# miloknowles/adaptive-stereo-icra-2021

Measured on AMD Instinct MI355X. Metric: stereo pairs/sec (fwd+adapt-step), KITTI 1242x375 D=192, higher is better.
Workload: dtype f32

## Files before the change

adaptive-stereo-icra-2021_amd/adaptive_stereo/_native.py:

```python
import ctypes
import os

import torch

_HERE = os.path.dirname(os.path.abspath(__file__))
LIB_PATH = os.path.join(_HERE, "libadaptive_stereo_hip.so")
BUILD_HINT = "build it with: make -C %s" % os.path.join(os.path.dirname(_HERE), "csrc")

c_int, c_float, c_i64, c_vp = ctypes.c_int, ctypes.c_float, ctypes.c_int64, ctypes.c_void_p


class Pcl(ctypes.Structure):
  _fields_ = [(n, ctypes.c_int32) for n in ("B", "D", "H", "W", "pd", "ph", "pw")]

  def numel(self):
    return self.B * (self.D + 2 * self.pd) * (self.H + 2 * self.ph) * (self.W + 2 * self.pw) * 32

  def voxels(self):
    return self.B * self.D * self.H * self.W

  def key(self):
    return (self.B, self.D, self.H, self.W, self.pd, self.ph, self.pw)


# ... 4 lines not shown
    return self.kd * self.kh * self.kw


class BnMerge(ctypes.Structure):
  _fields_ = [(n, c_vp) for n in ("stat_mean", "stat_m2", "stat_cnt", "gamma", "beta", "running_mean", "running_var",
                                 "save_mean", "save_invstd", "scale", "shift")] + \
             [("nparts", ctypes.c_int32), ("momentum", c_float), ("eps", c_float)]


class TrunkBn(ctypes.Structure):
  _fields_ = [(n, c_vp) for n in ("stat_mean", "stat_m2", "stat_cnt", "gamma", "beta", "state")] + \
             [("nparts", ctypes.c_int32), ("eps", c_float)]


_P = ctypes.POINTER
_SIGNATURES = {
  "as_last_error": (ctypes.c_char_p, []),
  "as_version": (c_int, []),
  "as_pcl_numel": (c_i64, [_P(Pcl)]),
  "as_cost_volume_fwd": (c_int, [c_vp, c_vp, c_vp, _P(Pcl), c_vp]),
  "as_cost_volume_bwd": (c_int, [c_vp, c_vp, c_vp, _P(Pcl), c_vp]),
  "as_conv32_pack_weights": (c_int, [c_vp, c_vp, _P(ConvShape), c_int, c_vp]),
  "as_conv32_pack_weights_batch": (c_int, [c_vp, c_int, c_int, c_vp]),
  "as_conv32_num_blocks": (c_int, [_P(Pcl)]),
  "as_conv32_stat_parts": (c_int, [_P(Pcl), _P(Pcl), _P(ConvShape)]),
  "as_conv32_fwd": (c_int, [c_vp, _P(Pcl), c_vp, c_vp, c_vp, _P(Pcl), _P(ConvShape), c_int, c_vp, c_vp, c_float,
                            c_vp, c_vp, c_vp, c_vp, c_vp]),
  "as_conv32_dgrad_s2_workspace": (c_i64, []),
  "as_conv32_dgrad_s2": (c_int, [c_vp, _P(Pcl), c_vp, c_vp, _P(Pcl), c_vp, c_vp]),
  "as_conv32_dgrad_s2_pack": (c_int, [c_vp, c_vp, c_vp]),
  "as_conv32_dgrad_s2_packed": (c_int, [c_vp, _P(Pcl), c_vp, c_vp, _P(Pcl), c_vp]),
  "as_conv32_wgrad_workspace": (c_i64, [_P(Pcl), _P(Pcl), _P(ConvShape)]),
  "as_conv32_wgrad": (c_int, [c_vp, _P(Pcl), c_vp, _P(Pcl), _P(ConvShape), c_vp, c_vp, c_int, c_vp, c_vp]),
  "as_bn_finalize": (c_int, [c_vp, c_vp, c_vp, c_int, c_vp, c_vp, c_vp, c_vp, c_float, c_float, c_vp, c_vp, c_vp,
                             c_vp, c_vp]),
  "as_bn_eval_affine": (c_int, [c_vp, c_vp, c_vp, c_vp, c_float, c_vp, c_vp, c_vp, c_vp, c_vp]),
  "as_bn_eval_affine_batch": (c_int, [c_vp, c_int, c_float, c_vp]),
  "as_bn_act_fwd": (c_int, [c_vp, c_vp, c_vp, c_float, c_vp, c_vp, _P(Pcl), c_vp]),
  "as_bn_bwd_workspace": (c_i64, [_P(Pcl)]),
  "as_bn_act_bwd": (c_int, [c_vp, c_vp, c_vp, c_vp, c_vp, c_vp, c_vp, c_float, c_int, c_vp, c_vp, c_vp, c_int, c_vp,
                            _P(Pcl), c_vp]),
  "as_bn_act_bwd_given": (c_int, [c_vp, c_vp, c_vp, c_vp, c_vp, c_vp, c_vp, c_float, c_int, c_vp, c_vp, c_vp, c_int, c_vp,
                                  _P(Pcl), c_int, c_vp]),
  "as_bn_bwd_coef_offset": (c_i64, []),
  "as_bn_bwd_sums": (c_int, [c_vp, c_vp, c_vp, c_vp, c_vp, c_float, c_vp, _P(Pcl), c_int, c_vp, c_vp]),
  "as_bn_bwd_finalize_synced": (c_int, [c_vp, c_vp, c_vp, c_vp, c_vp, c_vp, c_int, c_vp, c_vp]),
  "as_bn_bwd_apply": (c_int, [c_vp, c_vp, c_vp, c_vp, c_vp, c_float, c_vp, c_vp, _P(Pcl), c_vp]),
  "as_conv32_wgrad_bnapply_ok": (c_int, [_P(Pcl), _P(Pcl), _P(ConvShape)]),
  "as_conv32_wgrad_bnapply": (c_int, [c_vp, _P(Pcl), c_vp, c_vp, _P(Pcl), _P(ConvShape), c_vp, c_vp, c_vp, c_vp, c_float,
                                      c_vp, c_vp, c_vp, c_int, c_vp, c_vp]),
  "as_conv32to1_bnsums_ok": (c_int, [_P(Pcl), _P(ConvShape)]),
  "as_conv32to1_bnsums_parts": (c_int, [_P(Pcl)]),
  "as_conv32to1_dgrad_bnsums": (c_int, [c_vp, _P(Pcl), _P(ConvShape), c_vp, c_vp, c_vp, c_vp, c_vp, c_vp, c_float, c_vp, c_vp]),
  "as_wgrad_defer": (c_int, [c_int]),
  "as_wgrad_defer_pending": (c_int, []),
  "as_wgrad_defer_flush": (c_int, [c_vp]),
  "as_conv32_act_ok": (c_int, [_P(Pcl), _P(Pcl), _P(ConvShape)]),
  "as_conv32_act_parts": (c_int, []),
  "as_conv32_act_fwd": (c_int, [c_vp, c_vp, c_vp, c_vp, c_vp, _P(Pcl), c_vp, c_vp, c_float, c_vp, _P(Pcl), _P(ConvShape), c_vp, c_vp,
                                c_vp, c_vp]),
  "as_conv32_wino_ok": (c_int, [_P(Pcl), _P(Pcl), _P(ConvShape)]),
  "as_conv32_wino_parts": (c_int, []),
  "as_conv32_wino_pack_weights": (c_int, [c_vp, c_vp, c_int, c_vp]),
  "as_conv32_wino_fwd": (c_int, [c_vp, c_vp, c_vp, c_vp, c_vp, _P(Pcl), c_vp, c_vp, c_float, c_vp, _P(Pcl), _P(ConvShape), c_vp, c_vp,
                                 c_vp, c_vp]),
  "as_conv32_wino_eval": (c_int, [c_vp, _P(Pcl), _P(ConvShape), c_vp, c_vp, c_vp, c_vp, c_float, c_int, c_vp, c_vp]),
  "as_conv32_wino_bwd_data": (c_int, [c_vp, c_vp, _P(Pcl), _P(ConvShape), c_vp, c_vp, c_vp, c_vp, c_vp, c_float, c_vp, c_vp, c_vp, c_vp,
                                      c_vp, c_vp, c_vp, c_vp]),
  "as_conv32_wino_bwd_filter": (c_int, [c_vp, c_vp, _P(Pcl), _P(ConvShape), c_vp, c_vp, c_int, c_vp, c_vp]),
  "as_conv32_wino_bwd_parts": (c_int, []),
  "as_conv32_wino_bwd_workspace": (c_i64, []),
  "as_conv32_wino_bwd_generation": (c_int, [c_int]),
  "as_conv32_wino_bwd": (c_int, [c_vp, _P(Pcl), c_vp, c_vp, _P(Pcl), _P(ConvShape), c_vp, c_vp, c_vp, c_vp, c_vp, c_float, c_vp,
                                 c_vp, c_vp, c_vp, c_vp, c_vp, c_vp, c_vp, c_int, c_vp, c_vp, c_vp]),
  "as_conv32_wino_bwd_fused_parts": (c_int, []),
  "as_conv32_wino_bwd_fused_workspace": (c_i64, []),
  "as_conv32_wino_bwd_fused": (c_int, [c_vp, _P(Pcl), c_vp, c_vp, _P(Pcl), _P(ConvShape), c_vp, c_vp, c_vp, c_vp, c_vp, c_float, c_vp,
                                       c_vp, c_vp, c_vp, c_vp, c_vp, c_vp, c_int, c_vp, c_vp, c_vp]),
  "as_conv3d_wgrad_lds_assignment": (c_int, [c_int, c_int, c_int, c_vp, c_vp, c_vp]),
  "as_conv32_s2_enable": (c_int, [c_int]),
  "as_conv4_s2_enable": (c_int, [c_int]),
  "as_refine_out_ok": (c_int, [_P(Pcl)]),
  "as_refine_out_fwd": (c_int, [c_vp, c_vp, c_vp, c_vp, c_float, c_vp, _P(Pcl), c_vp, c_vp, c_vp, c_int, c_vp, c_vp]),
  "as_conv32_bwd_fused_ok": (c_int, [_P(Pcl), _P(Pcl), _P(ConvShape)]),
  "as_conv32_bwd_fused_parts": (c_int, []),
  "as_conv32_bwd_fused_workspace": (c_i64, []),
  "as_conv32_bwd_fused": (c_int, [c_vp, _P(Pcl), c_vp, c_vp, _P(Pcl), _P(ConvShape), c_vp, c_vp, c_vp, c_vp, c_vp, c_float, c_vp, c_vp,
                                  c_vp, c_vp, c_vp, c_vp, c_vp, c_int, c_vp, c_vp, c_vp]),
  "as_conv32_bnbwd_parts": (c_int, [_P(Pcl), _P(Pcl), _P(ConvShape)]),
  "as_conv32_fwd_bnbwd": (c_int, [c_vp, _P(Pcl), c_vp, c_vp, _P(Pcl), _P(ConvShape), c_vp, c_vp, c_vp, c_vp, c_vp, c_float,
                                  c_vp, c_vp]),
  "as_agg3d_ok": (c_int, [_P(Pcl)]),
  "as_agg3d_parts": (c_int, [_P(Pcl)]),
  "as_agg3d_fwd": (c_int, [c_vp, _P(Pcl), c_vp, c_vp, c_vp, c_vp, _P(BnMerge), c_vp, c_vp, c_int, c_vp, c_vp, c_float, c_vp, c_vp,
                           c_vp, c_vp]),
  "as_trunk_parts": (c_int, [_P(Pcl), c_int]),
  "as_trunk_fwd": (c_int, [c_vp, c_vp, _P(TrunkBn), c_vp, _P(Pcl), c_int, c_vp, c_vp, c_float, c_vp, c_vp, c_vp, c_vp, c_vp]),
  "as_trunk_finish_fwd": (c_int, [c_vp, _P(Pcl), c_vp, c_vp, c_int, c_int, _P(c_vp), _P(c_vp), c_float, c_vp]),
  "as_trunk_begin_bwd": (c_int, [c_vp, c_vp, c_int, _P(Pcl), c_vp, c_vp]),
  "as_trunk_bwd_workspace": (c_i64, [_P(Pcl), c_int]),
  "as_trunk_bwd": (c_int, [c_vp, c_vp, c_vp, c_vp, c_int, c_vp, c_vp, c_vp, c_vp, c_vp, c_vp, c_vp, c_vp, _P(Pcl), c_int, c_float,
                           c_vp, c_vp, c_int, c_vp, c_vp]),
  "as_trunk_finish_bwd": (c_int, [c_vp, c_int, c_int, _P(c_vp), _P(c_vp), c_int, c_vp]),
  "as_agg_tail_ok": (c_int, [_P(Pcl)]),
  "as_agg_tail_fwd": (c_int, [c_vp, _P(Pcl), c_vp, c_vp, _P(BnMerge), c_vp, c_vp, c_vp, c_float, c_vp, c_vp, c_vp, c_vp, c_vp]),
  "as_conv3d_out_fwd": (c_int, [c_vp, _P(Pcl), c_vp, c_vp, c_vp, c_vp]),
  "as_conv3d_out_bwd_workspace": (c_i64, [_P(Pcl)]),
  "as_conv3d_out_bwd": (c_int, [c_vp, c_vp, _P(Pcl), c_vp, c_vp, c_vp, c_vp, c_int, c_vp, c_vp]),
  "as_conv32to1_fwd": (c_int, [c_vp, _P(Pcl), _P(ConvShape), c_vp, c_vp, c_vp, c_int, c_vp, c_vp]),
  "as_conv32to1_bwd_workspace": (c_i64, [_P(Pcl), _P(ConvShape)]),
  "as_conv32to1_bwd": (c_int, [c_vp, c_vp, _P(Pcl), _P(ConvShape), c_vp, c_vp, c_vp, c_vp, c_int, c_vp, c_vp]),
  "as_pcl4_numel": (c_i64, [_P(Pcl)]),
  "as_pack_in4": (c_int, [c_vp, c_vp, c_int, c_vp, _P(Pcl), c_vp]),
  "as_conv4_pack_weights": (c_int, [c_vp, c_int, c_vp, _P(ConvShape), c_vp]),
  "as_conv4_wgrad_bnapply_ok": (c_int, [_P(Pcl), _P(Pcl), _P(ConvShape)]),
  "as_conv4_wgrad_bnapply_proj": (c_int, [c_vp, _P(Pcl), c_vp, c_vp, _P(Pcl), _P(ConvShape), c_int, c_vp, c_vp, c_vp, c_vp, c_float,
                                          c_vp, c_vp, c_vp, c_vp, c_int, c_vp, c_vp]),
  "as_tap_gather": (c_int, [c_vp, c_vp, c_vp, c_int, c_int, c_int, c_vp]),
  "as_conv4_wgrad_bnapply": (c_int, [c_vp, _P(Pcl), c_vp, c_vp, _P(Pcl), _P(ConvShape), c_int, c_vp, c_vp, c_vp, c_vp, c_float,
                                     c_vp, c_vp, c_vp, c_int, c_vp, c_vp]),
  "as_conv4_stat_parts": (c_int, [_P(Pcl), _P(Pcl), _P(ConvShape)]),
  "as_conv4_fwd": (c_int, [c_vp, _P(Pcl), c_vp, c_vp, c_vp, _P(Pcl), _P(ConvShape), c_int, c_vp, c_vp, c_float,
                           c_vp, c_vp, c_vp, c_vp]),
  "as_conv4_wgrad_workspace": (c_i64, [_P(Pcl), _P(ConvShape)]),
  "as_conv4_wgrad": (c_int, [c_vp, _P(Pcl), c_vp, _P(Pcl), _P(ConvShape), c_int, c_vp, c_vp, c_int, c_vp, c_vp]),
  "as_softargmax_fwd": (c_int, [c_vp, c_int, c_int, c_int, c_int, c_vp, c_vp, c_vp, c_vp]),
  "as_softargmax_bwd": (c_int, [c_vp, c_vp, c_vp, c_int, c_int, c_int, c_int, c_vp, c_vp]),
  "as_agg_tail_bwd_ok": (c_int, [_P(Pcl)]),
  "as_agg_tail_bwd_workspace": (c_i64, [_P(Pcl)]),
  "as_agg_tail_bwd": (c_int, [c_vp, c_vp, c_vp, c_vp, _P(Pcl), c_vp, c_vp, c_vp, c_vp, c_int, c_vp, c_vp]),
  "as_upsample_bilinear_fwd": (c_int, [c_vp, c_int, c_int, c_int, c_vp, c_int, c_int, c_float, c_vp]),
  "as_upsample_bilinear_bwd": (c_int, [c_vp, c_int, c_int, c_int, c_vp, c_int, c_int, c_float, c_vp]),
  "as_warp_fwd": (c_int, [c_vp, c_vp, c_int, c_int, c_int, c_int, c_int, c_vp, c_vp, c_vp]),
  "as_warp_nearest_fwd": (c_int, [c_vp, c_vp, c_int, c_int, c_int, c_int, c_int, c_vp, c_vp, c_vp]),
  "as_warp_bwd": (c_int, [c_vp, c_vp, c_vp, c_int, c_int, c_int, c_int, c_int, c_vp, c_vp]),
  "as_warp_bwd_add": (c_int, [c_vp, c_vp, c_vp, c_vp, c_int, c_int, c_int, c_int, c_int, c_vp, c_vp]),
  "as_monodepth_loss_bwd_masked": (c_int, [c_vp, c_vp, c_vp, c_vp, c_vp, c_vp, c_vp, c_int, c_int, c_int, c_float, c_vp, c_vp, c_vp,
                                           c_vp, c_vp]),
  "as_monodepth_workspace": (c_i64, [c_int, c_int, c_int]),
  "as_monodepth_loss_fwd": (c_int, [c_vp, c_vp, c_vp, c_int, c_int, c_int, c_float, c_vp, c_vp, c_vp, c_vp, c_vp,
                                    c_vp]),
  "as_monodepth_loss_bwd": (c_int, [c_vp, c_vp, c_vp, c_vp, c_vp, c_vp, c_vp, c_int, c_int, c_int, c_float, c_vp,
                                    c_vp, c_vp, c_vp]),
  "as_photometric_chain_workspace": (c_i64, [c_int, c_int, c_int]),
  "as_photometric_chain_fwd": (c_int, [c_vp, c_vp, c_vp, c_int, c_int, c_int, c_float, c_vp, c_vp, c_vp, c_vp, c_vp]),
  "as_photometric_chain_bwd": (c_int, [c_vp, c_vp, c_vp, c_vp, c_vp, c_vp, c_int, c_int, c_int, c_float, c_vp, c_vp, c_vp, c_vp]),
  "as_monodepth_loss_rows_fwd": (c_int, [c_vp, c_vp, c_vp, c_int, c_int, c_int, c_float, c_vp, c_vp, c_vp, c_vp, c_vp, c_vp]),
  "as_masked_sum_workspace": (c_i64, [c_i64]),
  "as_masked_sum": (c_int, [c_vp, c_vp, c_i64, c_vp, c_vp, c_vp]),
  "as_masked_sum_mean": (c_int, [c_vp, c_vp, c_i64, c_vp, c_vp, c_vp]),
  "as_khamis_workspace": (c_i64, [c_i64]),
  "as_khamis_fwd": (c_int, [c_vp, c_vp, c_i64, c_vp, c_vp, c_vp]),
  "as_khamis_bwd": (c_int, [c_vp, c_vp, c_vp, c_vp, c_i64, c_vp, c_vp]),
  "as_eval_metrics_workspace": (c_i64, [c_i64]),
  "as_eval_metrics": (c_int, [c_vp, c_vp, c_i64, c_vp, c_vp, c_vp]),
  "as_relu_bwd": (c_int, [c_vp, c_vp, c_i64, c_vp, c_vp]),
  "as_mirror_taps_ch0": (c_int, [c_vp, c_int, c_vp, c_vp, c_vp]),
  "as_sumsq_workspace": (c_i64, [c_i64]),
  "as_clip_coef": (c_int, [c_vp, c_float, c_vp, c_vp]),
  "as_sumsq_clip": (c_int, [c_vp, c_i64, c_float, c_vp, c_vp, c_vp, c_vp, c_vp]),
  "as_sumsq": (c_int, [c_vp, c_i64, c_vp, c_vp, c_vp]),
  "as_adam_step": (c_int, [c_vp, c_vp, c_vp, c_vp, c_i64, c_vp, c_float, c_float, c_float, c_float, c_int, c_vp,
                           c_vp]),
  "as_decode_rgb8": (c_int, [c_vp, c_int, c_int, c_int, c_int, c_int, c_int, c_int, c_vp, c_vp]),
  "as_decode_plane": (c_int, [c_vp, c_int, c_int, c_int, c_int, c_int, c_int, c_int, c_int, c_int, c_float, c_int, c_vp,
                              c_vp]),
# ... 62 lines not shown
```

adaptive-stereo-icra-2021_amd/adaptive_stereo/hip_ops.py:

```python
import os
import torch

from . import _native as nat
from ._native import Pcl, ConvShape, call, ptr, stream, f32c

LEAKY_SLOPE = 0.2
BN_EPS = 1e-5
BN_MOMENTUM = 0.1

CONV3D_333 = ConvShape(3, 3, 3, 1, 1, 1, 1, 1)

_DIRECT_GRADS = True


def set_direct_grad_accumulation(flag: bool):
  global _DIRECT_GRADS
  _DIRECT_GRADS = bool(flag)


def grad_sinks(params):
  if not (_DIRECT_GRADS and torch.is_grad_enabled()):
    return None
  out = []
  for p in params:
# ... 52 lines not shown

  def put(self, buf, g: Pcl, channels=32):
    if buf is None:
      return
    self.free.setdefault(self._key(buf.device, g, channels), []).append(buf)

  def clear(self):
    self.free.clear()


POOL = PclPool()


class _RmwOrder(object):
  enabled = False
  last = {}
  streams = {}


def rmw_order_reset(enabled):
  if not enabled:
    flush_deferred_reductions()
  _RmwOrder.enabled = bool(enabled)
  _RmwOrder.last = {}
  _RmwOrder.streams = {}
  if enabled and _DEFER_REDUCE and torch.cuda.is_available():
    lib = nat.load()
    if lib.as_wgrad_defer_pending() != 0 or _DeferredReduce.keep:
      raise RuntimeError("adaptive_stereo: a multi-stream region opens while weight-gradient reductions of an earlier one "
                         "are still pending (a region was left without rmw_order_reset(False))")
    _DeferredReduce.on = True
    lib.as_wgrad_defer(1)


class _DeferredReduce(object):
  on = False
  keep = []


_DEFER_REDUCE = True


def set_defer_reduce(enabled):
  global _DEFER_REDUCE
  prev, _DEFER_REDUCE = _DEFER_REDUCE, bool(enabled)
  return prev


def _keep_for_deferred_reduce(ws):
  if _DeferredReduce.on:
    _DeferredReduce.keep.append(ws)


def flush_deferred_reductions():
  join_region_streams()
  if not _DeferredReduce.on:
    return
  lib = nat.load()
  lib.as_wgrad_defer(0)
  _DeferredReduce.on = False
  call("as_wgrad_defer_flush", stream())
  _DeferredReduce.keep = []


_TAIL_BNSUMS = True
_HEAD_PROJ = True
_FWD_ACT = True
_WINOGRAD = os.environ.get("AS_DIAG_DIRECT_FORM") != "1"


def set_tail_bnsums(enabled):
  global _TAIL_BNSUMS
  prev, _TAIL_BNSUMS = _TAIL_BNSUMS, bool(enabled)
  return prev


def set_head_proj(enabled):
  global _HEAD_PROJ
  prev, _HEAD_PROJ = _HEAD_PROJ, bool(enabled)
  return prev


_REFINE_OUT = True


def set_refine_out(enabled):
  global _REFINE_OUT
  prev, _REFINE_OUT = _REFINE_OUT, bool(enabled)
  return prev


def set_head_staged(enabled):
  lib = nat.load()
  prev = lib.as_conv32_s2_enable(2) == 1 and lib.as_conv4_s2_enable(2) == 1
  lib.as_conv32_s2_enable(1 if enabled else 0)
  lib.as_conv4_s2_enable(1 if enabled else 0)
  return prev


def set_fwd_act(enabled):
  global _FWD_ACT
  prev, _FWD_ACT = _FWD_ACT, bool(enabled)
  return prev


_WINOGRAD_BWD = True
_WINOGRAD_BWD_ONE_LAUNCH = True


def set_winograd_bwd_one_launch(flag: bool):
  global _WINOGRAD_BWD_ONE_LAUNCH
  prev, _WINOGRAD_BWD_ONE_LAUNCH = _WINOGRAD_BWD_ONE_LAUNCH, bool(flag)
  return prev


def set_winograd(enabled, backward=None):
  global _WINOGRAD, _WINOGRAD_BWD
  prev, _WINOGRAD = _WINOGRAD, bool(enabled)
  _WINOGRAD_BWD = bool(enabled if backward is None else backward)
  return prev


class _Beside(object):
  enabled = os.environ.get("AS_WGRAD_BESIDE", "0") == "1"
  stream = None
  origin = None
  forks = 0


def set_wgrad_beside(flag: bool):
  prev, _Beside.enabled = _Beside.enabled, bool(flag)
  return prev


def set_fork_origin(handle):
  prev, _Beside.origin = _Beside.origin, handle
  return prev


def fork_beside(fn):
  main = torch.cuda.current_stream()
  if (not _Beside.enabled or _BN_SYNC is not None or
      (torch.cuda.is_current_stream_capturing() and main.cuda_stream != _Beside.origin)):
    fn()
    return None
  if _Beside.stream is None:
    _Beside.stream = torch.cuda.Stream()
  side = _Beside.stream
  side.wait_stream(main)
  with torch.cuda.stream(side):
    fn()
  ev = torch.cuda.Event()
  ev.record(side)
  _Beside.forks += 1
  return ev


def join_beside(ev):
  if ev is not None:
    torch.cuda.current_stream().wait_event(ev)


def _rmw_wait(t):
  if _RmwOrder.enabled and t is not None:
    last = _RmwOrder.last.get(t.data_ptr())
    cur = torch.cuda.current_stream()
    if last is not None and last[0] != cur.cuda_stream:
      cur.wait_event(last[1])


def _rmw_done(t):
# ... 1034 lines not shown
           ptr(stats.mean), ptr(stats.m2), ptr(stats.cnt), stream())
      st0 = bn_train_stats(stats, gamma0, beta0, rm0, rv0)
      fused_act = _FWD_ACT and need_bwd and all(lib.as_conv32_act_ok(g, g, conv_shape_2d(d)) == 1 for d in REFINE_DILATIONS)
      a0 = None if fused_act else bn_act(z0, st0, g)
    else:
      fused_act = False
      st0 = bn_eval_stats(gamma0, beta0, rm0, rv0)
      if need_bwd:
        z0 = POOL.get(g, dev)
        call("as_conv4_fwd", ptr(in4), g4, ptr(wp4), ptr(b0), ptr(z0), g, s33, 0, None, None, LEAKY_SLOPE, None, None,
             None, stream())
        a0 = bn_act(z0, st0, g)
      else:
        z0 = None
        a0 = POOL.get(g, dev)
        call("as_conv4_fwd", ptr(in4), g4, ptr(wp4), ptr(b0), ptr(a0), g, s33, 1, ptr(st0.scale), ptr(st0.shift),
             LEAKY_SLOPE, None, None, None, stream())
    if not need_bwd and z0 is not None:
      POOL.put(z0, g); z0 = None

    xs, zs, sts = [a0], [], []
    tail_fused = None
    if fused_act:
      xs = []
      z_prev, st_prev = z0, st0
      for l, dil in enumerate(REFINE_DILATIONS):
        wl, bl, gamma, beta = params[4 + 4 * l:8 + 4 * l]
        rm, rv = bn_buffers[1 + l]
        a_prev, z, st = block_forward_act(z_prev, xs[-1] if xs else None, st_prev, g, conv_shape_2d(dil), wl, bl, gamma, beta,
                                          rm, rv)
        xs.append(a_prev); zs.append(z); sts.append(st)
        z_prev, st_prev = z, st
      if _REFINE_OUT and lib.as_refine_out_ok(g) == 1:
        tail_fused = (z_prev, xs[-1], st_prev)
      else:
        xs.append(bn_act(z_prev, st_prev, g, residual=xs[-1]))
    else:
      for l, dil in enumerate(REFINE_DILATIONS):
        wl, bl, gamma, beta = params[4 + 4 * l:8 + 4 * l]
        rm, rv = bn_buffers[1 + l]
        z, a, st = block_forward(xs[-1], g, conv_shape_2d(dil), wl, bl, gamma, beta, rm, rv, train, True, need_bwd)
        zs.append(z); sts.append(st); xs.append(a)
        if not need_bwd:
          POOL.put(xs[-2], g)

    w_out, b_out = params[28], params[29]
    out = torch.empty(B, 1, H, W, dtype=torch.float32, device=dev)
    if tail_fused is not None:
      z6, a5, st6 = tail_fused
      a6 = POOL.get(g, dev)
      call("as_refine_out_fwd", ptr(z6), ptr(a5), ptr(st6.scale), ptr(st6.shift), LEAKY_SLOPE, ptr(a6), g, ptr(w_out), ptr(b_out),
           ptr(up), 1, ptr(out), stream())
      xs.append(a6)
    elif _REFINE_OUT and lib.as_refine_out_ok(g) == 1:
      call("as_refine_out_fwd", ptr(xs[-1]), None, None, None, LEAKY_SLOPE, None, g, ptr(w_out), ptr(b_out), ptr(up), 1, ptr(out),
           stream())
    else:
      call("as_conv32to1_fwd", ptr(xs[-1]), g, s33, ptr(w_out), ptr(b_out), ptr(up), 1, ptr(out), stream())

    if need_bwd:
      ctx.g, ctx.g4, ctx.train = g, g4, bool(train)
      ctx.sinks = sinks
      ctx.dims = (B, h, w, H, W, float(gain))
      ctx.in4, ctx.z0, ctx.st0 = in4, z0, st0
      ctx.xs, ctx.zs, ctx.sts = xs, zs, sts
      ctx.save_for_backward(out, *params)
    else:
      POOL.put(xs[-1], g); POOL.put(in4, g4, channels=4)
    return out

  @staticmethod
  def backward(ctx, g_out):
    out, *params = ctx.saved_tensors
    g, g4 = ctx.g, ctx.g4
    B, h, w, H, W, gain = ctx.dims
    dev = out.device
    lib = nat.load()
    s33 = conv_shape_2d(1)
    xs, zs, sts = ctx.xs, ctx.zs, ctx.sts
    grads = [None] * 30

    g_out = f32c(g_out)
    g_pre = torch.empty_like(out)
    call("as_relu_bwd", ptr(g_out), ptr(out), out.numel(), ptr(g_pre), stream())
    w_out = params[28]
    sinks = ctx.sinks
    g_a = POOL.get(g, dev)
    ws = _empty(lib.as_conv32to1_bwd_workspace(g, s33), dev)
    sums = None
    if _sink(sinks, 28) is not None and _sink(sinks, 29) is not None:
      if _TAIL_BNSUMS and ctx.train and _BN_SYNC is None and lib.as_conv32to1_bnsums_ok(g, s33) == 1:
        nws = _empty(lib.as_bn_bwd_workspace(g), dev)
        ev = fork_beside(lambda: call("as_conv32to1_bwd", ptr(g_pre), ptr(xs[6]), g, s33, ptr(w_out), None, ptr(sinks[28]),
                                      ptr(sinks[29]), 1, ptr(ws), stream()))
        call("as_conv32to1_dgrad_bnsums", ptr(g_pre), g, s33, ptr(w_out), ptr(g_a), ptr(zs[5]), ptr(sts[5].scale),
             ptr(sts[5].shift), ptr(sts[5].mean), LEAKY_SLOPE, ptr(nws), stream())
        join_beside(ev)
        sums = BnBwdSums(nws, lib.as_conv32to1_bnsums_parts(g))
      else:
        call("as_conv32to1_bwd", ptr(g_pre), ptr(xs[6]), g, s33, ptr(w_out), ptr(g_a), ptr(sinks[28]), ptr(sinks[29]), 1,
             ptr(ws), stream())
    else:
      g_wout, g_bout = torch.empty_like(w_out), _empty(1, dev)
      call("as_conv32to1_bwd", ptr(g_pre), ptr(xs[6]), g, s33, ptr(w_out), ptr(g_a), ptr(g_wout), ptr(g_bout), 0,
           ptr(ws), stream())
      grads[28], grads[29] = g_wout, g_bout

    for l in range(5, -1, -1):
      wl, bl, gamma, beta = params[4 + 4 * l:8 + 4 * l]
      next_bn = (zs[l - 1], sts[l - 1]) if l > 0 else (ctx.z0, ctx.st0)
      g_x, dW, db, g_gamma, g_beta, sums = block_backward(g_a, xs[l], zs[l], sts[l], wl, gamma, g,
                                                          conv_shape_2d(REFINE_DILATIONS[l]), ctx.train, True, True,
                                                          sinks[4 + 4 * l:8 + 4 * l] if sinks is not None else None,
                                                          sums, next_bn)
      grads[4 + 4 * l:8 + 4 * l] = [dW, db, g_gamma, g_beta]
      POOL.put(g_a, g); POOL.put(zs[l], g); POOL.put(xs[l + 1], g)
      g_a = g_x

    w0, b0, gamma0, beta0 = params[0:4]
    ws4 = _empty(lib.as_conv4_wgrad_workspace(g, s33), dev)
    all_sinks = all(_sink(sinks, i) is not None for i in range(4))
    if all_sinks and lib.as_conv4_wgrad_bnapply_ok(g4, g, s33) == 1:
      bws = sums.workspace if sums is not None else _empty(lib.as_bn_bwd_workspace(g), dev)
      st0 = ctx.st0
      bn_bwd_coefs(g_a, ctx.z0, st0, gamma0, g, ctx.train, sinks[2], sinks[3], True, bws, sums)
      coef = bws[lib.as_bn_bwd_coef_offset():]
      if _HEAD_PROJ and ctx.needs_input_grad[0] and not ctx.needs_input_grad[1]:
        w_proj = pack_special(w0, PACK_MIRROR_TAP, 9, 288,
                              lambda w_, o_: call("as_mirror_taps_ch0", ptr(w_), 4, ptr(o_), None, stream()))
        h_proj = _empty(B * 9 * H * W, dev)
        call("as_conv4_wgrad_bnapply_proj", ptr(ctx.in4), g4, ptr(g_a), ptr(ctx.z0), g, s33, 4, ptr(st0.scale), ptr(st0.shift),
             ptr(st0.mean), ptr(coef), LEAKY_SLOPE, ptr(w_proj), ptr(h_proj), ptr(sinks[0]), ptr(sinks[1]), 1, ptr(ws4),
             stream())
        g_z0 = None
      else:
        h_proj = None
        g_z0 = POOL.get(g, dev)
        call("as_conv4_wgrad_bnapply", ptr(ctx.in4), g4, ptr(g_a), ptr(ctx.z0), g, s33, 4, ptr(st0.scale), ptr(st0.shift),
             ptr(st0.mean), ptr(coef), LEAKY_SLOPE, ptr(g_z0), ptr(sinks[0]), ptr(sinks[1]), 1, ptr(ws4), stream())
      dW0 = db0 = g_gamma0 = g_beta0 = None
    else:
      h_proj = None
      g_z0, g_gamma0, g_beta0 = bn_act_bwd(g_a, ctx.z0, ctx.st0, gamma0, g, ctx.train, _sink(sinks, 2), _sink(sinks, 3), sums)
      if _sink(sinks, 0) is not None and _sink(sinks, 1) is not None:
        call("as_conv4_wgrad", ptr(ctx.in4), g4, ptr(g_z0), g, s33, 4, ptr(sinks[0]), ptr(sinks[1]), 1, ptr(ws4), stream())
        dW0 = db0 = None
      else:
        dW0 = torch.empty_like(w0); db0 = _empty(32, dev)
        call("as_conv4_wgrad", ptr(ctx.in4), g4, ptr(g_z0), g, s33, 4, ptr(dW0), ptr(db0), 0, ptr(ws4), stream())
    grads[0:4] = [dW0, db0, g_gamma0, g_beta0]

    g_coarse = None
    if ctx.needs_input_grad[0]:
      g_up = torch.empty(B, 1, H, W, dtype=torch.float32, device=dev)
      if h_proj is not None:
        call("as_tap_gather", ptr(h_proj), ptr(g_pre), ptr(g_up), B, H, W, stream())
      else:
        w_ch0 = pack_special(w0, PACK_MIRROR_CH, 9, 288,
                             lambda w_, o_: call("as_mirror_taps_ch0", ptr(w_), 4, None, ptr(o_), stream()))
        call("as_conv32to1_fwd", ptr(g_z0), g, s33, ptr(w_ch0), None, ptr(g_pre), 0, ptr(g_up), stream())
      g_coarse = torch.empty(B, h, w, dtype=torch.float32, device=dev)
      call("as_upsample_bilinear_bwd", ptr(g_up), B, H, W, ptr(g_coarse), h, w, gain, stream())
    if ctx.needs_input_grad[1]:
      raise NotImplementedError("EdgeRefineFn: gradient w.r.t. the guidance image is not part of the adaptation path")
    POOL.put(g_z0, g); POOL.put(g_a, g); POOL.put(ctx.z0, g); POOL.put(xs[0], g); POOL.put(ctx.in4, g4, channels=4)
    ctx.xs = ctx.zs = ctx.sts = ctx.in4 = ctx.z0 = None
    return (g_coarse, None, None, None, None, None) + tuple(grads)


class UpsampleBilinearFn(torch.autograd.Function):

  @staticmethod
  def forward(ctx, src, H, W, gain):
    src = f32c(src)
    B, h, w = src.shape
    dst = torch.empty(B, 1, H, W, dtype=torch.float32, device=src.device)
    call("as_upsample_bilinear_fwd", ptr(src), B, h, w, ptr(dst), int(H), int(W), float(gain), stream())
    ctx.dims = (B, h, w, int(H), int(W), float(gain))
    return dst

  @staticmethod
  def backward(ctx, g_dst):
    B, h, w, H, W, gain = ctx.dims
    g_dst = f32c(g_dst)
    g_src = torch.empty(B, h, w, dtype=torch.float32, device=g_dst.device)
    call("as_upsample_bilinear_bwd", ptr(g_dst), B, H, W, ptr(g_src), h, w, gain, stream())
    return g_src, None, None, None


# ... 179 lines not shown
```

adaptive-stereo-icra-2021_amd/csrc/refine_out.hip:

```cpp
#include "as_common.h"

#define RO_COLS 126
#ifndef RO_ROWS_ACT
#define RO_ROWS_ACT 32
#endif
#ifndef RO_ROWS_PLAIN
#define RO_ROWS_PLAIN 12
#endif
#define RO_PW 132

struct RefineOutArgs {
  const float* x;
  const float* skip;
  const float* scale;
  const float* shift;
  float* a_out;
  const float* w;
  const float* bias;
  const float* add_src;
  float* out;
  PclDev g;
  int nseg, nstrips, relu;
  float slope;
};
// ... 51 lines not shown
    const bool row_own = yi >= ya && yi < yb;
#pragma unroll
    for (int k = 0; k < 4; ++k) {
      f32x4 y = rz[k];
      if (ACT) {
        y = y * sc + sh;
        y.x = y.x > 0.f ? y.x : y.x * p.slope; y.y = y.y > 0.f ? y.y : y.y * p.slope;
        y.z = y.z > 0.f ? y.z : y.z * p.slope; y.w = y.w > 0.f ? y.w : y.w * p.slope;
        if (p.skip) y += rs[k];
      }
      if (!row_in || !((colmask >> k) & 1u)) y = (f32x4){0.f, 0.f, 0.f, 0.f};
      *reinterpret_cast<f32x4*>(xrow + lds_w + k * 4096) = y;
      if (ACT && row_own && ((ownmask >> k) & 1u))
        *reinterpret_cast<f32x4*>(p.a_out + row0 + (long)yi * p.g.Wp * 32 + k * 1024) = y;
    }
    if (yi < yb) fetch(yi + 1, rz, rs);
    __syncthreads();
    f32x16 acc;
    {
      f32x4 xa[4];
#pragma unroll
      for (int q = 0; q < 4; ++q) xa[q] = *reinterpret_cast<const f32x4*>(a_rd + (((4 * h + q) ^ a_sw) << 4));
      const f32x16 zero = {0.f, 0.f, 0.f, 0.f, 0.f, 0.f, 0.f, 0.f, 0.f, 0.f, 0.f, 0.f, 0.f, 0.f, 0.f, 0.f};
      acc = __builtin_amdgcn_mfma_f32_32x32x2f32(xa[0].x, Bw[0], zero, 0, 0, 0);
      acc = __builtin_amdgcn_mfma_f32_32x32x2f32(xa[0].y, Bw[1], acc, 0, 0, 0);
      acc = __builtin_amdgcn_mfma_f32_32x32x2f32(xa[0].z, Bw[2], acc, 0, 0, 0);
      acc = __builtin_amdgcn_mfma_f32_32x32x2f32(xa[0].w, Bw[3], acc, 0, 0, 0);
#pragma unroll
      for (int q = 1; q < 4; ++q) {
        acc = __builtin_amdgcn_mfma_f32_32x32x2f32(xa[q].x, Bw[4 * q + 0], acc, 0, 0, 0);
        acc = __builtin_amdgcn_mfma_f32_32x32x2f32(xa[q].y, Bw[4 * q + 1], acc, 0, 0, 0);
        acc = __builtin_amdgcn_mfma_f32_32x32x2f32(xa[q].z, Bw[4 * q + 2], acc, 0, 0, 0);
        acc = __builtin_amdgcn_mfma_f32_32x32x2f32(xa[q].w, Bw[4 * q + 3], acc, 0, 0, 0);
      }
    }
    if (li < 9) {
      float* pr = &P[(yi + 1) % 3][li][32 * wave + 4 * h];
#pragma unroll
      for (int r = 0; r < 16; ++r) pr[(r & 3) + 8 * (r >> 2)] = acc[r];
    }
    __syncthreads();
    const int yo = yi - 1;
    if (yo >= ya && t < RO_COLS && x0 + t < W) {
      float s = bias;
#pragma unroll
      for (int ky = 0; ky < 3; ++ky) {
        const float (*pr)[RO_PW] = P[(yo + ky) % 3];
#pragma unroll
        for (int kx = 0; kx < 3; ++kx) s += pr[ky * 3 + kx][t + kx];
      }
      const long o = ((long)b * H + yo) * W + x0 + t;
      if (p.add_src) s += p.add_src[o];
      if (p.relu) s = s > 0.f ? s : 0.f;
      p.out[o] = s;
    }
  }
}

extern "C" int as_refine_out_ok(const as_pcl* g) {
  if (!as_pcl_ok(g)) return 0;
  return g->D == 1 && g->pd == 0 && g->ph >= 1 && g->pw >= 1 && (long)g->ph * (g->W + 2 * g->pw) >= 128 ? 1 : 0;
}

extern "C" int as_refine_out_fwd(const float* x, const float* skip, const float* scale, const float* shift, float slope,
                                 float* a_out, const as_pcl* g, const float* w, const float* bias, const float* add_src,
                                 int relu, float* out, void* stream) {
  AS_CHECK_ARG(as_refine_out_ok(g) == 1, "as_refine_out_fwd: geometry not supported (as_refine_out_ok() == 0)");
  AS_CHECK_ARG(x && w && out, "as_refine_out_fwd: null pointer");
  AS_CHECK_ARG((scale == nullptr) == (shift == nullptr) && (scale == nullptr) == (a_out == nullptr),
               "as_refine_out_fwd: scale, shift and a_out come together (the fused BatchNorm + LeakyReLU) or not at all");
  AS_CHECK_ARG(scale != nullptr || skip == nullptr, "as_refine_out_fwd: a skip connection needs the fused activation");
  AS_CHECK_ARG(a_out == nullptr || (a_out != x && a_out != skip), "as_refine_out_fwd: a_out must not alias an input");
  AS_CHECK_ARG(scale == nullptr || (slope > 0.f && slope < 1.f), "as_refine_out_fwd: slope must lie in (0, 1)");
  RefineOutArgs a;
  a.x = x; a.skip = skip; a.scale = scale; a.shift = shift; a.a_out = a_out; a.w = w; a.bias = bias; a.add_src = add_src;
  a.out = out; a.g = as_make_dev(g); a.relu = relu; a.slope = slope;
  a.nseg = as_div_up(g->W, RO_COLS); a.nstrips = as_div_up(g->H, scale ? RO_ROWS_ACT : RO_ROWS_PLAIN);
  const int grid = g->B * a.nseg * a.nstrips;
  if (scale) hipLaunchKernelGGL(refine_out_kernel<true>, dim3(grid), dim3(256), 0, (hipStream_t)stream, a);
  else hipLaunchKernelGGL(refine_out_kernel<false>, dim3(grid), dim3(256), 0, (hipStream_t)stream, a);
  AS_CHECK_LAUNCH("as_refine_out_fwd");
  return AS_OK;
}
```

include/adaptive_stereo_hip.h:

```cpp
#ifndef ADAPTIVE_STEREO_HIP_H_
#define ADAPTIVE_STEREO_HIP_H_

#include <stdint.h>

#ifdef __cplusplus
extern "C" {
#endif

#define AS_CHANNELS 32
#define AS_MAX_TAPS 32

typedef struct as_pcl {
  int32_t B, D, H, W;
  int32_t pd, ph, pw;
} as_pcl;

typedef struct as_conv_shape {
  int32_t kd, kh, kw;
  int32_t pad_d, pad_h, pad_w;
  int32_t dil;
  int32_t stride;
} as_conv_shape;

const char* as_last_error(void);
// ... 7 lines not shown
                           int transpose_flip, void* stream);

typedef struct as_pack_job {
  const float* w;
  float* packed;
  int32_t taps;
  int32_t transpose_flip;
} as_pack_job;
#define AS_PACK_S2_DGRAD 2
#define AS_PACK_CONV4 16
#define AS_PACK_MIRROR_TAP 32
#define AS_PACK_MIRROR_CH 33
#define AS_PACK_WINO 34
#define AS_PACK_WINO_T 35
int as_conv32_pack_weights_batch(const as_pack_job* jobs, int njobs, int max_taps, void* stream);
int as_conv32_num_blocks(const as_pcl* gout);
int as_conv32_stat_parts(const as_pcl* gin, const as_pcl* gout, const as_conv_shape* s);
int as_conv32_fwd(const float* x, const as_pcl* gin, const float* packed_w, const float* bias,
                  float* z, const as_pcl* gout, const as_conv_shape* s,
                  int epilogue, const float* ep_scale, const float* ep_shift, float slope,
                  const float* residual, float* stat_mean, float* stat_m2, float* stat_cnt, void* stream);
int as_conv32_bwd_fused_ok(const as_pcl* gin, const as_pcl* gout, const as_conv_shape* s);
int as_conv32_bwd_fused_parts(void);
int64_t as_conv32_bwd_fused_workspace(void);
int as_conv32_bwd_fused(const float* x, const as_pcl* gin, const float* g_a, const float* z, const as_pcl* gout,
                        const as_conv_shape* s, const float* packed_wt, const float* scale, const float* shift,
                        const float* mean, const float* coef, float slope, const float* next_z,
                        const float* next_scale, const float* next_shift, const float* next_mean, float* g_x,
                        float* dW, float* db, int accumulate, float* next_bn_workspace, float* workspace, void* stream);

int as_wgrad_defer(int on);
int as_wgrad_defer_pending(void);
int as_wgrad_defer_flush(void* stream);

int as_conv32_act_ok(const as_pcl* gin, const as_pcl* gout, const as_conv_shape* s);
int as_conv32_act_parts(void);
int as_conv32_act_fwd(const float* z_prev, const float* a_prevprev, const float* in_scale, const float* in_shift,
                      float* a_out, const as_pcl* gin, const float* packed_w, const float* bias, float slope,
                      float* z, const as_pcl* gout, const as_conv_shape* s, float* stat_mean, float* stat_m2,
                      float* stat_cnt, void* stream);

int as_conv32_wino_ok(const as_pcl* gin, const as_pcl* gout, const as_conv_shape* s);
int as_conv32_wino_parts(void);
int as_conv32_wino_pack_weights(const float* w, float* packed, int transposed, void* stream);
int as_conv32_wino_fwd(const float* z_prev, const float* a_prevprev, const float* in_scale, const float* in_shift,
                       float* a_out, const as_pcl* gin, const float* wino_w, const float* bias, float slope,
                       float* z, const as_pcl* gout, const as_conv_shape* s, float* stat_mean, float* stat_m2,
                       float* stat_cnt, void* stream);

int as_conv32_wino_eval(const float* x, const as_pcl* g, const as_conv_shape* s, const float* wino_w, const float* bias,
                        const float* scale, const float* shift, float slope, int residual, float* out, void* stream);

int as_conv32_wino_bwd_parts(void);
int64_t as_conv32_wino_bwd_workspace(void);
int as_conv32_wino_bwd_generation(int generation);
int as_conv32_wino_bwd_data(const float* g_a, const float* z, const as_pcl* g, const as_conv_shape* s,
                            const float* wino_wt, const float* scale, const float* shift, const float* mean,
                            const float* coef, float slope, const float* next_z, const float* next_scale,
                            const float* next_shift, const float* next_mean, float* g_z, float* g_x,
                            float* next_bn_workspace, void* stream);
int as_conv32_wino_bwd_filter(const float* x, const float* g_z, const as_pcl* g, const as_conv_shape* s, float* dW,
                              float* db, int accumulate, float* workspace, void* stream);
int as_conv32_wino_bwd(const float* x, const as_pcl* gin, const float* g_a, const float* z, const as_pcl* gout,
                       const as_conv_shape* s, const float* wino_wt, const float* scale, const float* shift,
                       const float* mean, const float* coef, float slope, const float* next_z,
                       const float* next_scale, const float* next_shift, const float* next_mean, float* g_z,
                       float* g_x, float* dW, float* db, int accumulate, float* next_bn_workspace,
                       float* workspace, void* stream);
int as_conv32_wino_bwd_fused_parts(void);
int64_t as_conv32_wino_bwd_fused_workspace(void);
int as_conv32_wino_bwd_fused(const float* x, const as_pcl* gin, const float* g_a, const float* z, const as_pcl* gout,
                             const as_conv_shape* s, const float* wino_wt, const float* scale, const float* shift,
                             const float* mean, const float* coef, float slope, const float* next_z,
                             const float* next_scale, const float* next_shift, const float* next_mean, float* g_x,
                             float* dW, float* db, int accumulate, float* next_bn_workspace, float* workspace, void* stream);

int as_conv32_s2_enable(int on);
int as_conv4_s2_enable(int on);

int as_refine_out_ok(const as_pcl* g);
int as_refine_out_fwd(const float* x, const float* skip, const float* scale, const float* shift, float slope, float* a_out,
                      const as_pcl* g, const float* w, const float* bias, const float* add_src, int relu, float* out,
                      void* stream);

typedef struct as_bn_merge {
  const float* stat_mean;
  const float* stat_m2;
  const float* stat_cnt;
  const float* gamma;
  const float* beta;
  float* running_mean;
  float* running_var;
  float* save_mean;
  float* save_invstd;
  float* scale;
  float* shift;
  int32_t nparts;
  float momentum;
  float eps;
} as_bn_merge;
int as_agg3d_ok(const as_pcl* g);
int as_agg3d_parts(const as_pcl* g);
int as_agg3d_fwd(const float* x, const as_pcl* g, const float* packed_w, const float* bias,
                 const float* in_scale, const float* in_shift, const as_bn_merge* in_bn, float* a_out,
                 float* z, int epilogue, const float* ep_scale, const float* ep_shift, float slope,
                 float* stat_mean, float* stat_m2, float* stat_cnt, void* stream);

int as_agg_tail_ok(const as_pcl* g);
int as_agg_tail_fwd(const float* x, const as_pcl* g, const float* in_scale, const float* in_shift,
                    const as_bn_merge* in_bn, float* a_out,
                    const float* w, const float* bias, float slope, float* logits, float* pred,
                    int32_t* argmax, float* fcs, void* stream);

typedef struct as_trunk_bn {
  const float* stat_mean;
  const float* stat_m2;
  const float* stat_cnt;
  const float* gamma;
  const float* beta;
  float* state;
  int32_t nparts;
  float eps;
} as_trunk_bn;
int as_trunk_parts(const as_pcl* g, int ngroups);
int as_trunk_fwd(const float* src, const float* skip, const as_trunk_bn* bn_prev, float* a_out, const as_pcl* g, int ngroups,
                 const float* packed_w, const float* bias, float slope, float* z, float* stat_mean, float* stat_m2,
                 float* stat_cnt, void* stream);
int as_trunk_finish_fwd(const float* feats_pcl, const as_pcl* g, float* feats_nchw, const float* states, int nlayers,
                        int ngroups, float* const* running_mean, float* const* running_var, float momentum, void* stream);
int as_trunk_begin_bwd(const float* g_a, const float* g_b, int nA, const as_pcl* g, float* out_pcl, void* stream);
int64_t as_trunk_bwd_workspace(const as_pcl* g, int ngroups);
int as_trunk_bwd(const float* g_a, const float* z, const float* state, const double* sums, int nparts, const float* gamma,
                 float* bn_grads, const float* x, const float* packed_wt, float* g_x, const float* z_next,
                 const float* state_next, double* sums_next, const as_pcl* g, int ngroups, float slope, float* dW, float* db,
                 int accumulate, float* workspace, void* stream);
int as_trunk_finish_bwd(const float* bn_grads, int nlayers, int ngroups, float* const* g_gamma, float* const* g_beta,
                        int accumulate, void* stream);

int64_t as_conv32_dgrad_s2_workspace(void);
int as_conv32_dgrad_s2(const float* gz, const as_pcl* ggz, const float* w, float* gx, const as_pcl* ggx,
                       float* workspace, void* stream);
int as_conv32_dgrad_s2_pack(const float* w, float* packed, void* stream);
int as_conv32_dgrad_s2_packed(const float* gz, const as_pcl* ggz, const float* packed, float* gx, const as_pcl* ggx,
                              void* stream);
int64_t as_conv32_wgrad_workspace(const as_pcl* gin, const as_pcl* gout, const as_conv_shape* s);
int as_conv32_wgrad(const float* x, const as_pcl* gin, const float* gz, const as_pcl* gout,
                    const as_conv_shape* s, float* dW, float* db, int accumulate, float* workspace, void* stream);
int as_conv3d_wgrad_lds_assignment(int ntiles, int nchunks, int block, int* chunk, int* kd, int* extra_tile);

int as_bn_finalize(const float* stat_mean, const float* stat_m2, const float* stat_cnt, int nparts,
                   const float* gamma, const float* beta, float* running_mean, float* running_var,
                   float momentum, float eps, float* save_mean, float* save_invstd,
                   float* scale, float* shift, void* stream);
int as_bn_eval_affine(const float* gamma, const float* beta, const float* running_mean,
                      const float* running_var, float eps, float* save_mean, float* save_invstd,
                      float* scale, float* shift, void* stream);
typedef struct as_bn_affine_job {
  const float* gamma;
  const float* beta;
  const float* running_mean;
  const float* running_var;
  float* out;
} as_bn_affine_job;
int as_bn_eval_affine_batch(const as_bn_affine_job* jobs, int njobs, float eps, void* stream);
int as_bn_act_fwd(const float* z, const float* scale, const float* shift, float slope,
                  const float* residual, float* a, const as_pcl* g, void* stream);
// ... 155 lines not shown
```

Before: 602.5.

## Fuse refinement output backward: ReLU grad, dgrad, wgrad and BN sums in one kernel

Adds a HIP kernel that computes the ReLU backward of the refinement head output, the 32-to-1 3x3 conv data gradient, the weight/bias gradient partials and the BatchNorm backward sums in a single pass. It replaces a separate ReLU-backward launch plus two conv32to1 kernels that previously ran on forked streams. The goal is to avoid re-reading the activation and gradient tensors several times and to cut launch and stream-sync overhead. In exchange the fused kernel serialises the wgrad work with the dgrad work instead of overlapping them on a side stream.

```diff
diff --git a/adaptive-stereo-icra-2021_amd/adaptive_stereo/_native.py b/adaptive-stereo-icra-2021_amd/adaptive_stereo/_native.py
--- a/adaptive-stereo-icra-2021_amd/adaptive_stereo/_native.py
+++ b/adaptive-stereo-icra-2021_amd/adaptive_stereo/_native.py
@@ -110,6 +110,8 @@
   "as_conv4_s2_enable": (c_int, [c_int]),
   "as_refine_out_ok": (c_int, [_P(Pcl)]),
   "as_refine_out_fwd": (c_int, [c_vp, c_vp, c_vp, c_vp, c_float, c_vp, _P(Pcl), c_vp, c_vp, c_vp, c_int, c_vp, c_vp]),
+  "as_refine_out_bwd": (c_int, [c_vp, c_vp, c_vp, c_vp, _P(Pcl), c_vp, c_vp, c_vp, c_vp, c_float, c_vp, c_vp, c_vp, c_vp,
+                                c_vp, c_int, c_vp, c_vp]),
   "as_conv32_bwd_fused_ok": (c_int, [_P(Pcl), _P(Pcl), _P(ConvShape)]),
   "as_conv32_bwd_fused_parts": (c_int, []),
   "as_conv32_bwd_fused_workspace": (c_i64, []),
diff --git a/adaptive-stereo-icra-2021_amd/adaptive_stereo/hip_ops.py b/adaptive-stereo-icra-2021_amd/adaptive_stereo/hip_ops.py
--- a/adaptive-stereo-icra-2021_amd/adaptive_stereo/hip_ops.py
+++ b/adaptive-stereo-icra-2021_amd/adaptive_stereo/hip_ops.py
@@ -158,11 +158,18 @@
 
 
 _REFINE_OUT = True
+_REFINE_OUT_BWD = True
 
 
 def set_refine_out(enabled):
   global _REFINE_OUT
   prev, _REFINE_OUT = _REFINE_OUT, bool(enabled)
+  return prev
+
+
+def set_refine_out_bwd(enabled):
+  global _REFINE_OUT_BWD
+  prev, _REFINE_OUT_BWD = _REFINE_OUT_BWD, bool(enabled)
   return prev
 
 
@@ -1363,29 +1370,37 @@
 
     g_out = f32c(g_out)
     g_pre = torch.empty_like(out)
-    call("as_relu_bwd", ptr(g_out), ptr(out), out.numel(), ptr(g_pre), stream())
     w_out = params[28]
     sinks = ctx.sinks
     g_a = POOL.get(g, dev)
     ws = _empty(lib.as_conv32to1_bwd_workspace(g, s33), dev)
     sums = None
-    if _sink(sinks, 28) is not None and _sink(sinks, 29) is not None:
-      if _TAIL_BNSUMS and ctx.train and _BN_SYNC is None and lib.as_conv32to1_bnsums_ok(g, s33) == 1:
-        nws = _empty(lib.as_bn_bwd_workspace(g), dev)
-        ev = fork_beside(lambda: call("as_conv32to1_bwd", ptr(g_pre), ptr(xs[6]), g, s33, ptr(w_out), None, ptr(sinks[28]),
-                                      ptr(sinks[29]), 1, ptr(ws), stream()))
-        call("as_conv32to1_dgrad_bnsums", ptr(g_pre), g, s33, ptr(w_out), ptr(g_a), ptr(zs[5]), ptr(sts[5].scale),
-             ptr(sts[5].shift), ptr(sts[5].mean), LEAKY_SLOPE, ptr(nws), stream())
-        join_beside(ev)
-        sums = BnBwdSums(nws, lib.as_conv32to1_bnsums_parts(g))
+    with_sinks = _sink(sinks, 28) is not None and _sink(sinks, 29) is not None
+    tail_sums = _TAIL_BNSUMS and ctx.train and _BN_SYNC is None and lib.as_conv32to1_bnsums_ok(g, s33) == 1
+    if with_sinks and tail_sums and _REFINE_OUT_BWD:
+      nws = _empty(lib.as_bn_bwd_workspace(g), dev)
+      call("as_refine_out_bwd", ptr(g_out), ptr(out), ptr(xs[6]), ptr(zs[5]), g, ptr(w_out), ptr(sts[5].scale), ptr(sts[5].shift),
+           ptr(sts[5].mean), LEAKY_SLOPE, ptr(g_pre), ptr(g_a), ptr(nws), ptr(sinks[28]), ptr(sinks[29]), 1, ptr(ws), stream())
+      sums = BnBwdSums(nws, lib.as_conv32to1_bnsums_parts(g))
+    else:
+      call("as_relu_bwd", ptr(g_out), ptr(out), out.numel(), ptr(g_pre), stream())
+      if with_sinks:
+        if tail_sums:
+          nws = _empty(lib.as_bn_bwd_workspace(g), dev)
+          ev = fork_beside(lambda: call("as_conv32to1_bwd", ptr(g_pre), ptr(xs[6]), g, s33, ptr(w_out), None, ptr(sinks[28]),
+                                        ptr(sinks[29]), 1, ptr(ws), stream()))
+          call("as_conv32to1_dgrad_bnsums", ptr(g_pre), g, s33, ptr(w_out), ptr(g_a), ptr(zs[5]), ptr(sts[5].scale),
+               ptr(sts[5].shift), ptr(sts[5].mean), LEAKY_SLOPE, ptr(nws), stream())
+          join_beside(ev)
+          sums = BnBwdSums(nws, lib.as_conv32to1_bnsums_parts(g))
+        else:
+          call("as_conv32to1_bwd", ptr(g_pre), ptr(xs[6]), g, s33, ptr(w_out), ptr(g_a), ptr(sinks[28]), ptr(sinks[29]), 1,
+               ptr(ws), stream())
       else:
-        call("as_conv32to1_bwd", ptr(g_pre), ptr(xs[6]), g, s33, ptr(w_out), ptr(g_a), ptr(sinks[28]), ptr(sinks[29]), 1,
+        g_wout, g_bout = torch.empty_like(w_out), _empty(1, dev)
+        call("as_conv32to1_bwd", ptr(g_pre), ptr(xs[6]), g, s33, ptr(w_out), ptr(g_a), ptr(g_wout), ptr(g_bout), 0,
              ptr(ws), stream())
-    else:
-      g_wout, g_bout = torch.empty_like(w_out), _empty(1, dev)
-      call("as_conv32to1_bwd", ptr(g_pre), ptr(xs[6]), g, s33, ptr(w_out), ptr(g_a), ptr(g_wout), ptr(g_bout), 0,
-           ptr(ws), stream())
-      grads[28], grads[29] = g_wout, g_bout
+        grads[28], grads[29] = g_wout, g_bout
 
     for l in range(5, -1, -1):
       wl, bl, gamma, beta = params[4 + 4 * l:8 + 4 * l]
diff --git a/adaptive-stereo-icra-2021_amd/csrc/refine_out.hip b/adaptive-stereo-icra-2021_amd/csrc/refine_out.hip
--- a/adaptive-stereo-icra-2021_amd/csrc/refine_out.hip
+++ b/adaptive-stereo-icra-2021_amd/csrc/refine_out.hip
@@ -157,3 +157,151 @@
   AS_CHECK_LAUNCH("as_refine_out_fwd");
   return AS_OK;
 }
+
+struct RefineOutBwdArgs {
+  const float* g_out;
+  const float* out;
+  const float* a;
+  const float* z;
+  const float* w;
+  const float* bn_scale; const float* bn_shift; const float* bn_mean;
+  float slope;
+  float* g_pre;
+  float* g_a;
+  double* bn_partial;
+  float* w_partial;
+  PclDev g;
+  int nchunks, chunks_per_row;
+};
+
+__global__ __launch_bounds__(256, 4) void refine_out_bwd_kernel(RefineOutBwdArgs p) {
+  __shared__ float sg[2][3][132];
+  __shared__ float red[2][32][33];
+  __shared__ f32x4 wl[9][8];
+  const int c4 = threadIdx.x & 7, vl = threadIdx.x >> 3;
+  const int H = p.g.H, W = p.g.W;
+  if (threadIdx.x < 72) {
+    const int k = threadIdx.x >> 3;
+    wl[k][c4] = (f32x4){p.w[(c4 * 4 + 0) * 9 + k], p.w[(c4 * 4 + 1) * 9 + k], p.w[(c4 * 4 + 2) * 9 + k], p.w[(c4 * 4 + 3) * 9 + k]};
+  }
+  const f32x4 bsc = *reinterpret_cast<const f32x4*>(p.bn_scale + c4 * 4), bsh = *reinterpret_cast<const f32x4*>(p.bn_shift + c4 * 4);
+  const f32x4 bmu = *reinterpret_cast<const f32x4*>(p.bn_mean + c4 * 4);
+  f32x4 s_dy = {0.f, 0.f, 0.f, 0.f}, s_dx = {0.f, 0.f, 0.f, 0.f};
+  f32x4 acc[9];
+#pragma unroll
+  for (int k = 0; k < 9; ++k) acc[k] = (f32x4){0.f, 0.f, 0.f, 0.f};
+  float gsum = 0.f;
+  const int i0 = threadIdx.x, i1 = threadIdx.x + 256;
+  const int r0 = i0 / 130, q0 = i0 - r0 * 130, r1 = i1 / 130, q1 = i1 - r1 * 130;
+  int it = 0;
+  for (int ch = blockIdx.x; ch < p.nchunks; ch += gridDim.x, it ^= 1) {
+    const int rowi = ch / p.chunks_per_row, cx = ch - rowi * p.chunks_per_row;
+    const int y = rowi % H, b = rowi / H, x0 = cx * 128;
+    const int nf4 = min(128, W - x0) * 8;
+    auto gload = [&](int r, int c, float& go, float& o) {
+      const int yy = y - 1 + r, xx = x0 - 1 + c;
+      const long i = ((long)b * H + min(max(yy, 0), H - 1)) * W + min(max(xx, 0), W - 1);
+      go = p.g_out[i]; o = p.out[i];
+    };
+    float go0, o0, go1, o1;
+    gload(r0, q0, go0, o0);
+    gload(min(r1, 2), q1, go1, o1);
+    const long voff = (((long)b * p.g.Hp + (y + p.g.ph)) * p.g.Wp + (x0 + p.g.pw)) * 32;
+    f32x4 av[4], zv[4];
+#pragma unroll
+    for (int k4 = 0; k4 < 4; ++k4) {
+      const int f = min((int)threadIdx.x + 256 * k4, nf4 - 1);
+      av[k4] = *reinterpret_cast<const f32x4*>(p.a + voff + f * 4);
+      zv[k4] = *reinterpret_cast<const f32x4*>(p.z + voff + f * 4);
+    }
+    auto gstage = [&](int r, int c, float go, float o) {
+      const int yy = y - 1 + r, xx = x0 - 1 + c;
+      const float v = o > 0.f ? go : 0.f;
+      sg[it][r][c] = (yy >= 0 && yy < H && xx >= 0 && xx < W) ? v : 0.f;
+      if (r == 1 && c >= 1 && c <= 128 && xx < W) p.g_pre[((long)b * H + y) * W + xx] = v;
+    };
+    gstage(r0, q0, go0, o0);
+    if (i1 < 3 * 130) gstage(r1, q1, go1, o1);
+    __syncthreads();
+    const float (*sgc)[132] = sg[it];
+    float* dst = p.g_a + voff;
+#pragma unroll
+    for (int k4 = 0; k4 < 4; ++k4) {
+      const int f = threadIdx.x + 256 * k4;
+      if (f < nf4) {
+        const int vx = f >> 3;
+        if (c4 == 0) gsum += sgc[1][vx + 1];
+        f32x4 ga = {0.f, 0.f, 0.f, 0.f};
+#pragma unroll
+        for (int ky = 0; ky < 3; ++ky)
+#pragma unroll
+          for (int kx = 0; kx < 3; ++kx) {
+            const float gv = sgc[2 - ky][vx + 2 - kx];
+            ga += gv * wl[ky * 3 + kx][c4];
+            acc[ky * 3 + kx] += gv * av[k4];
+          }
+        *reinterpret_cast<f32x4*>(dst + f * 4) = ga;
+        const f32x4 yy = zv[k4] * bsc + bsh;
+        f32x4 gy;
+        gy.x = yy.x > 0.f ? ga.x : ga.x * p.slope; gy.y = yy.y > 0.f ? ga.y : ga.y * p.slope;
+        gy.z = yy.z > 0.f ? ga.z : ga.z * p.slope; gy.w = yy.w > 0.f ? ga.w : ga.w * p.slope;
+        s_dy += gy; s_dx += gy * (zv[k4] - bmu);
+      }
+    }
+  }
+  __syncthreads();
+  red[0][vl][c4 * 4 + 0] = s_dy.x; red[0][vl][c4 * 4 + 1] = s_dy.y; red[0][vl][c4 * 4 + 2] = s_dy.z; red[0][vl][c4 * 4 + 3] = s_dy.w;
+  red[1][vl][c4 * 4 + 0] = s_dx.x; red[1][vl][c4 * 4 + 1] = s_dx.y; red[1][vl][c4 * 4 + 2] = s_dx.z; red[1][vl][c4 * 4 + 3] = s_dx.w;
+  __syncthreads();
+  if (threadIdx.x < 64) {
+    const int which = threadIdx.x >> 5, c = threadIdx.x & 31;
+    double sum = 0.0;
+    for (int j = 0; j < 32; ++j) sum += (double)red[which][j][c];
+    p.bn_partial[(long)blockIdx.x * 64 + which * 32 + c] = sum;
+  }
+  float* wout = p.w_partial + (long)blockIdx.x * (9 * 32 + 1);
+#pragma unroll
+  for (int tp = 0; tp < 9; ++tp) {
+    __syncthreads();
+    red[0][vl][c4 * 4 + 0] = acc[tp].x; red[0][vl][c4 * 4 + 1] = acc[tp].y;
+    red[0][vl][c4 * 4 + 2] = acc[tp].z; red[0][vl][c4 * 4 + 3] = acc[tp].w;
+    __syncthreads();
+    if (threadIdx.x < 32) {
+      float s = 0.f;
+      for (int j = 0; j < 32; ++j) s += red[0][j][threadIdx.x];
+      wout[tp * 32 + threadIdx.x] = s;
+    }
+  }
+  __syncthreads();
+  if (c4 == 0) red[0][vl][0] = gsum;
+  __syncthreads();
+  if (threadIdx.x == 0) {
+    float s = 0.f;
+    for (int j = 0; j < 32; ++j) s += red[0][j][0];
+    wout[9 * 32] = s;
+  }
+}
+
+int as_conv32to1_wgrad_reduce(const float* partial, int nblocks, int ntaps, float* g_w, float* g_bias, int accumulate, hipStream_t st);
+
+extern "C" int as_refine_out_bwd(const float* g_out, const float* out, const float* a, const float* z, const as_pcl* g,
+                                 const float* w, const float* bn_scale, const float* bn_shift, const float* bn_mean, float slope,
+                                 float* g_pre, float* g_a, float* bn_workspace, float* g_w, float* g_bias, int accumulate,
+                                 float* workspace, void* stream) {
+  static const as_conv_shape s33 = {1, 3, 3, 0, 1, 1, 1, 1};
+  AS_CHECK_ARG(g && as_conv32to1_bnsums_ok(g, &s33) == 1, "as_refine_out_bwd: geometry not supported (as_conv32to1_bnsums_ok() != 1)");
+  AS_CHECK_ARG(g_out && out && a && z && w && bn_scale && bn_shift && bn_mean && g_pre && g_a && bn_workspace && g_w && g_bias &&
+               workspace, "as_refine_out_bwd: null pointer");
+  AS_CHECK_ARG(((uintptr_t)bn_workspace & 7) == 0, "as_refine_out_bwd: bn_workspace must be 8-byte aligned");
+  AS_CHECK_ARG(g_a != a && g_a != z && g_pre != g_out && g_pre != out, "as_refine_out_bwd: outputs must not alias inputs");
+  RefineOutBwdArgs q;
+  q.g_out = g_out; q.out = out; q.a = a; q.z = z; q.w = w; q.bn_scale = bn_scale; q.bn_shift = bn_shift; q.bn_mean = bn_mean;
+  q.slope = slope; q.g_pre = g_pre; q.g_a = g_a; q.bn_partial = reinterpret_cast<double*>(bn_workspace); q.w_partial = workspace;
+  q.g = as_make_dev(g);
+  q.chunks_per_row = (g->W + 127) / 128; q.nchunks = g->B * g->H * q.chunks_per_row;
+  const int grid = as_conv32to1_bnsums_parts(g);
+  hipStream_t st = (hipStream_t)stream;
+  hipLaunchKernelGGL(refine_out_bwd_kernel, dim3(grid), dim3(256), 0, st, q);
+  AS_CHECK_LAUNCH("as_refine_out_bwd");
+  return as_conv32to1_wgrad_reduce(workspace, grid, 9, g_w, g_bias, accumulate, st);
+}
diff --git a/include/adaptive_stereo_hip.h b/include/adaptive_stereo_hip.h
--- a/include/adaptive_stereo_hip.h
+++ b/include/adaptive_stereo_hip.h
@@ -113,6 +113,9 @@
 int as_refine_out_fwd(const float* x, const float* skip, const float* scale, const float* shift, float slope, float* a_out,
                       const as_pcl* g, const float* w, const float* bias, const float* add_src, int relu, float* out,
                       void* stream);
+int as_refine_out_bwd(const float* g_out, const float* out, const float* a, const float* z, const as_pcl* g, const float* w,
+                      const float* bn_scale, const float* bn_shift, const float* bn_mean, float slope, float* g_pre, float* g_a,
+                      float* bn_workspace, float* g_w, float* g_bias, int accumulate, float* workspace, void* stream);
 
 typedef struct as_bn_merge {
   const float* stat_mean;
```

Result: slower. 590.1 (median of 2 runs) (-2.1%).
